# Khrylx/EgoPose

Measured on AMD Instinct MI355X. Metric: env-steps/sec (whole node) ego_mimic PPO, higher is better.
Workload: dtype f64 (rollout kernels K1-K6, physics state) + f32 (policy/value nets)

## Files before the change

egopose_amd/_lib.py:

```python
from __future__ import annotations

import ctypes as C
import os

HERE = os.path.dirname(os.path.abspath(__file__))
LIB_PATH = os.path.join(HERE, "libegopose_hip.so")

EGP_OK = 0
EGP_EXPERT_ROW = 168

c_int_p = C.POINTER(C.c_int32)
c_dbl_p = C.POINTER(C.c_double)
vp = C.c_void_p


class ModelDesc(C.Structure):
    _fields_ = [
        ("nq", C.c_int32), ("nv", C.c_int32), ("nu", C.c_int32), ("nbody", C.c_int32), ("nM", C.c_int32),
        ("body_qpos_start", c_int_p), ("body_ndof", c_int_p), ("dof_parentid", c_int_p), ("dof_Madr", c_int_p),
        ("ee_body", c_int_p),
        ("jkp", c_dbl_p), ("jkd", c_dbl_p), ("a_ref", c_dbl_p), ("a_scale", c_dbl_p), ("torque_lim", c_dbl_p),
        ("b_diffw", c_dbl_p),
        ("sub_dt", C.c_double), ("frame_skip", C.c_int32), ("episode_len", C.c_int32),
        ("w_p", C.c_double), ("w_v", C.c_double), ("w_e", C.c_double), ("w_rp", C.c_double), ("w_rv", C.c_double),
# ... 32 lines not shown
class MlpLayer(C.Structure):
    _fields_ = [("wt", vp), ("bias", vp), ("in_dim", C.c_int32), ("out_dim", C.c_int32)]


class GemmDesc(C.Structure):
    _fields_ = [("M", C.c_int32), ("N", C.c_int32), ("K", C.c_int32),
                ("A", vp), ("lda", C.c_int64), ("a_kcontig", C.c_int32),
                ("B", vp), ("ldb", C.c_int64), ("b_kcontig", C.c_int32),
                ("C", vp), ("ldc", C.c_int64),
                ("bias", vp), ("relu", C.c_int32),
                ("mask", vp), ("ldmask", C.c_int64),
                ("terms", C.c_int32), ("splits", C.c_int32), ("accumulate", C.c_int32),
                ("bias_grad", vp), ("workspace", vp),
                ("a_rows", vp), ("A2", vp), ("lda2", C.c_int64), ("a_split", C.c_int32), ("a_src_rows", C.c_int64),
                ("b_krows", vp), ("B2", vp), ("ldb2", C.c_int64), ("b_split", C.c_int32), ("b_src_rows", C.c_int64),
                ("c_rows", vp), ("a_krows", vp)]


class PpoLossDesc(C.Structure):
    _fields_ = [("n", C.c_int32), ("n_pol", C.c_int32), ("act_dim", C.c_int32),
                ("rows", vp), ("pred", vp), ("returns", vp),
                ("mean", vp), ("ld_mean", C.c_int64),
                ("actions", vp), ("ld_act", C.c_int64),
                ("log_std", vp), ("adv", vp),
                ("fixed_logp", vp), ("write_fixed", C.c_int32),
                ("clip_eps", C.c_double), ("inv_n_val", C.c_double), ("inv_n_exp", C.c_double),
                ("d_pred", vp), ("d_mean", vp), ("ld_dmean", C.c_int64), ("d_log_std", vp),
                ("losses", vp), ("workspace", vp)]


class MinibatchPlanDesc(C.Structure):
# ... 248 lines not shown
```

egopose_amd/csrc/egp_gemm.hip:

```cpp
#include "egp_internal.hpp"

#include <type_traits>

namespace {

typedef __bf16 bf16x8 __attribute__((ext_vector_type(8)));
typedef __bf16 bf16x4 __attribute__((ext_vector_type(4)));
typedef float f32x16 __attribute__((ext_vector_type(16)));
typedef float f32x4u __attribute__((ext_vector_type(4), aligned(4)));
typedef float f32x4 __attribute__((ext_vector_type(4)));
typedef float f32x2 __attribute__((ext_vector_type(2)));

inline int after_launch(const char *what) {
    hipError_t e = hipGetLastError();
    if (e != hipSuccess) {
        egp::set_error("launch of %s failed: %s", what, hipGetErrorString(e));
        return EGP_E_HIP;
    }
    return EGP_OK;
}

constexpr int BM = 128, BK = 32;

#ifdef EGP_GEMM_TRACE
// ... 20 lines not shown
#else
#define EGP_TR(tag) do { } while (0)
#define EGP_TRW_DECL do { } while (0)
#define EGP_TRW(who, tag) do { } while (0)
#endif
__host__ __device__ constexpr int panel_el(int R) { return R * 8 + 32; }
__host__ __device__ constexpr int tile_el(int R) { return 4 * panel_el(R); }

struct GemmArgs {
    int M, N, K;
    const float *A; long lda; int a_kc;
    const float *B; long ldb; int b_kc;
    float *C; long ldc;
    const float *bias; int relu;
    const float *mask; long ldmask;
    int ones_col;
    int k_per_split;
    float *ws; int ldws;
    int tiles_m, tiles_n, xcd_order;
    int split_xcd;
    const long long *a_rows; const float *A2; long lda2; int a_split;
    const long long *a_krows;
    const long long *b_krows; const float *B2; long ldb2; int b_split;
    const long long *c_rows;
    int partial;
    int grid_tiles, n_items, zs;
};

template <int R, bool ktail>
__device__ __forceinline__ void load_kc(const float *__restrict__ P, long ld, int rows, int r0, int k0, int kend, float (&v)[R / 8],
// ... 247 lines not shown
#pragma unroll
    for (int i = 0; i < MI; ++i)
#pragma unroll
        for (int j = 0; j < NJ; ++j) {
            const int col = n0 + wn * 64 + 32 * j + (lane & 31);
            const int rbase = m0 + wm * WROWS + 32 * i + 4 * (lane >> 5);
            const int colc = min(col, n_out - 1);
            const float bv = (!partial && g.bias) ? g.bias[min(colc, g.N - 1)] : 0.f;
            float keep[16];
            if (!partial && g.mask) {
#pragma unroll
                for (int r = 0; r < 16; ++r) {
                    const int row = min(rbase + (r & 3) + 8 * (r >> 2), g.M - 1);
                    keep[r] = g.mask[(long)row * g.ldmask + min(colc, g.N - 1)];
                }
            } else {
#pragma unroll
                for (int r = 0; r < 16; ++r) keep[r] = 1.f;
            }
            if (interior) {
#pragma unroll
                for (int r = 0; r < 16; ++r) {
                    const int row = rbase + (r & 3) + 8 * (r >> 2);
                    float x = partial ? acc[i][j][r] : fmaxf(acc[i][j][r] + bv, floor_v);
                    x = keep[r] > 0.f ? x : 0.f;
                    dst[(long)row * ldd + col] = x;
                }
            } else {
#pragma unroll
                for (int r = 0; r < 16; ++r) {
                    const int row = rbase + (r & 3) + 8 * (r >> 2);
                    float x = partial ? acc[i][j][r] : fmaxf(acc[i][j][r] + bv, floor_v);
                    x = keep[r] > 0.f ? x : 0.f;
                    if (row < g.M && col < n_out) dst[(long)row * ldd + col] = x;
                }
            }
        }
    EGP_TR(21);
}

struct WsCursor {
    int w, s, nst;
    int m0, n0, z, kbeg, kend;
};

template <int BN>
__device__ __forceinline__ bool ws_item(const GemmArgs &g, int w, WsCursor &c) {
    const int L = w % g.grid_tiles, z = w / g.grid_tiles;
    int tm, tn;
// ... 366 lines not shown
                    f32x16 a = acc[i][j];
                    a = __builtin_amdgcn_mfma_f32_32x32x16_bf16(fb[ks][0][j], fa[ks][2][i], a, 0, 0, 0);
                    a = __builtin_amdgcn_mfma_f32_32x32x16_bf16(fb[ks][2][j], fa[ks][0][i], a, 0, 0, 0);
                    a = __builtin_amdgcn_mfma_f32_32x32x16_bf16(fb[ks][1][j], fa[ks][1][i], a, 0, 0, 0);
                    a = __builtin_amdgcn_mfma_f32_32x32x16_bf16(fb[ks][0][j], fa[ks][1][i], a, 0, 0, 0);
                    a = __builtin_amdgcn_mfma_f32_32x32x16_bf16(fb[ks][1][j], fa[ks][0][i], a, 0, 0, 0);
                    acc[i][j] = __builtin_amdgcn_mfma_f32_32x32x16_bf16(fb[ks][0][j], fa[ks][0][i], a, 0, 0, 0);
                }
    };
    constexpr int EP_LD = 64 + 4;
    float *patch = (float *)(smem + (size_t)2 * BUF_EL * sizeof(__bf16)) + wave * 32 * EP_LD;
    const bool partial = g.partial != 0;
    const int ncols = partial ? g.ldws : g.N;
    const long ldd = partial ? g.ldws : g.ldc;
    const float floor_v = g.relu ? 0.f : -__builtin_inff();
    auto epilogue_body = [&](auto partial_c, auto mask_c) __attribute__((always_inline)) {
        constexpr bool PARTIAL = decltype(partial_c)::value, MASK = decltype(mask_c)::value;
        float *dst = PARTIAL ? g.ws + (long)cur.z * g.M * g.ldws : g.C;
        const int col = cur.n0 + wn * 64 + 4 * (lane & 15);
        const int colc = min(col, ncols - 4);
        const bool col_ok = col < ncols;
        const int row0 = cur.m0 + wm * WROWS + (lane >> 4);
        long drow[MI][8];
#pragma unroll
        for (int i = 0; i < MI; ++i)
#pragma unroll
            for (int it = 0; it < 8; ++it) {
                const int row = row0 + 32 * i + 4 * it;
                drow[i][it] = (FUSED && !PARTIAL && g.c_rows) ? (long)g.c_rows[min(row, g.M - 1)] : (long)row;
            }
        f32x4u bv = {0.f, 0.f, 0.f, 0.f};
        if constexpr (!PARTIAL) bv = *(const f32x4u *)((g.bias ? g.bias : g.C) + colc);
        if (PARTIAL || !g.bias) bv = f32x4u{0.f, 0.f, 0.f, 0.f};
        f32x4u keep[MI][8];
        if constexpr (MASK) {
#pragma unroll
            for (int i = 0; i < MI; ++i)
#pragma unroll
                for (int it = 0; it < 8; ++it)
                    keep[i][it] = *(const f32x4u *)(g.mask + (long)min(row0 + 32 * i + 4 * it, g.M - 1) * g.ldmask + colc);
        }
#pragma unroll
        for (int i = 0; i < MI; ++i) {
#pragma unroll
            for (int j = 0; j < NJ; ++j)
#pragma unroll
                for (int rq = 0; rq < 4; ++rq)
                    *(float4 *)(patch + (lane & 31) * EP_LD + 32 * j + 8 * rq + 4 * (lane >> 5)) =
                        make_float4(acc[i][j][4 * rq], acc[i][j][4 * rq + 1], acc[i][j][4 * rq + 2], acc[i][j][4 * rq + 3]);
            __builtin_amdgcn_wave_barrier();
#pragma unroll
            for (int it = 0; it < 8; ++it) {
                const int row = row0 + 32 * i + 4 * it;
                float4 x = *(const float4 *)(patch + ((lane >> 4) + 4 * it) * EP_LD + 4 * (lane & 15));
                if constexpr (!PARTIAL) {
                    x.x = fmaxf(x.x + bv[0], floor_v); x.y = fmaxf(x.y + bv[1], floor_v);
                    x.z = fmaxf(x.z + bv[2], floor_v); x.w = fmaxf(x.w + bv[3], floor_v);
                }
                if constexpr (MASK) {
                    x.x = keep[i][it][0] > 0.f ? x.x : 0.f; x.y = keep[i][it][1] > 0.f ? x.y : 0.f;
                    x.z = keep[i][it][2] > 0.f ? x.z : 0.f; x.w = keep[i][it][3] > 0.f ? x.w : 0.f;
                }
                if (row < g.M && col_ok) *(f32x4u *)(dst + drow[i][it] * ldd + col) = f32x4u{x.x, x.y, x.z, x.w};
            }
            __builtin_amdgcn_wave_barrier();
        }
    };
    auto epilogue = [&]() __attribute__((always_inline)) {
        if (partial) epilogue_body(std::true_type{}, std::false_type{});
        else if (g.mask) epilogue_body(std::false_type{}, std::true_type{});
        else epilogue_body(std::false_type{}, std::false_type{});
    };
    clear();
    __syncthreads();
    for (int p = 0; p < P; ++p) {
        EGP_TRW(0, 40);
#if !defined(EGP_WS_SKIP) || EGP_WS_SKIP != 1
        compute(p & 1);
#endif
        EGP_TRW(0, 41);
        if (cur.s == cur.nst - 1) {
            epilogue();
            EGP_TRW(0, 43);
            clear();
            EGP_TRW(0, 42);
        }
        ws_next<BN>(g, cur, w_scan);
        __syncthreads();
    }
}

__global__ __launch_bounds__(256) void k_gemv_rows(GemmArgs g) {
    const int lane = threadIdx.x & 63, wave = threadIdx.x >> 6;
    const long bs = g.b_kc ? 1 : g.ldb;
    const float floor_v = g.relu ? 0.f : -__builtin_inff();
    for (long m = (long)blockIdx.x * 4 + wave; m < g.M; m += (long)gridDim.x * 4) {
        const float *__restrict__ a = g.A + m * g.lda;
        float acc = 0.f;
        for (int k = lane; k < g.K; k += 64) acc = fmaf(a[k], g.B[k * bs], acc);
#pragma unroll
        for (int off = 32; off > 0; off >>= 1) acc += __shfl_down(acc, off, 64);
        if (lane == 0) {
            float x = fmaxf(acc + (g.bias ? g.bias[0] : 0.f), floor_v);
            if (g.mask && !(g.mask[m * g.ldmask] > 0.f)) x = 0.f;
            g.C[m * g.ldc] = x;
        }
    }
}

__global__ __launch_bounds__(256) void k_rank1(GemmArgs g) {
    const long as = g.a_kc ? g.lda : 1, bs = g.b_kc ? g.ldb : 1;
    const float floor_v = g.relu ? 0.f : -__builtin_inff();
    const long total = (long)g.M * g.N;
    for (long id = (long)blockIdx.x * 256 + threadIdx.x; id < total; id += (long)gridDim.x * 256) {
        const long m = id / g.N;
        const int n = (int)(id - m * g.N);
        float x = fmaxf(fmaf(g.A[m * as], g.B[n * bs], g.bias ? g.bias[n] : 0.f), floor_v);
        if (g.mask && !(g.mask[m * g.ldmask + n] > 0.f)) x = 0.f;
        g.C[m * g.ldc + n] = x;
    }
}

__global__ __launch_bounds__(256) void k_colsum(GemmArgs g) {
    __shared__ float s_part[4][256 + 4];
    const int lane = threadIdx.x & 63, wave = threadIdx.x >> 6, z = blockIdx.x;
    const long as = g.a_kc ? 1 : g.lda;
    const int kbeg = z * g.k_per_split, kend = min(g.K, kbeg + g.k_per_split);
    const int n_out = g.N + (g.ones_col ? 1 : 0);
    float *__restrict__ dst = g.ws + (long)z * g.ldws;
    for (int n0 = 0; n0 < g.N; n0 += 256) {
        float acc[4] = {0.f, 0.f, 0.f, 0.f};
        for (int k = kbeg + wave; k < kend; k += 32) {
            float a[8];
#pragma unroll
// ... 146 lines not shown
    if (splits <= 1 && !ones_col) return 0;
    return (int64_t)(splits < 1 ? 1 : splits) * M * ((N + (ones_col ? 1 : 0) + 3) & ~3);
}

int egp_gemm_f32(const egp_gemm_desc *d, void *stream) {
    EGP_REQUIRE(d, "descriptor is NULL");
    EGP_REQUIRE(d->M >= 0 && d->N >= 0 && d->K >= 0, "negative size");
    EGP_REQUIRE(d->terms == 1 || d->terms == 3 || d->terms == 6, "terms must be 1 (bf16), 3 (two-piece split) or 6 (three-piece split)");
    if (d->M == 0 || d->N + (d->bias_grad ? 1 : 0) == 0) return EGP_OK;
    EGP_REQUIRE(d->A && d->B && d->C, "NULL operand");
    const int ones = d->bias_grad ? 1 : 0;
    const int splits = d->splits < 1 ? 1 : d->splits;
    const bool partial = splits > 1 || ones;
    EGP_REQUIRE(!partial || d->workspace, "split-K / bias-gradient launches need a workspace (egp_gemm_workspace_floats)");
    EGP_REQUIRE(!partial || (!d->bias && !d->relu && !d->mask), "no epilogue on split-K launches");
    EGP_REQUIRE(!d->accumulate || partial, "accumulate goes with split-K / bias-gradient launches only (a plain product would overwrite C)");
    EGP_REQUIRE(!ones || !d->b_kcontig, "the ones column (bias gradient) goes with B given as [k][n]");
    hipStream_t s = (hipStream_t)stream;
    GemmArgs g;
    g.M = d->M; g.N = d->N; g.K = d->K;
    g.A = d->A; g.lda = d->lda; g.a_kc = d->a_kcontig;
    g.B = d->B; g.ldb = d->ldb; g.b_kc = d->b_kcontig;
    g.C = d->C; g.ldc = d->ldc;
    g.bias = d->bias; g.relu = d->relu; g.mask = d->mask; g.ldmask = d->ldmask;
    g.ones_col = ones; g.ws = d->workspace; g.ldws = (d->N + ones + 3) & ~3; g.partial = partial ? 1 : 0;
    g.a_rows = (const long long *)d->a_rows; g.A2 = d->A2; g.lda2 = d->lda2; g.a_split = d->a_split;
    g.b_krows = (const long long *)d->b_krows; g.B2 = d->B2; g.ldb2 = d->ldb2; g.b_split = d->b_split;
    g.c_rows = (const long long *)d->c_rows;
    g.a_krows = (const long long *)d->a_krows;
    const bool fused_io = d->a_rows || d->A2 || d->b_krows || d->B2 || d->c_rows || d->a_krows;
    if (fused_io) {
        EGP_REQUIRE(!(d->a_rows || d->A2) || d->a_kcontig, "a_rows / A2 go with a k-contiguous A");
        EGP_REQUIRE(!(d->b_krows || d->B2) || !d->b_kcontig, "b_krows / B2 go with B given as [k][n]");
        EGP_REQUIRE(!d->a_krows || !d->a_kcontig, "a_krows goes with A given as [k][m]");
        EGP_REQUIRE(!d->A2 || (d->a_split > 0 && d->a_split % BK == 0 && d->K - d->a_split >= BK),
                    "a_split must be a multiple of 32 and leave at least 32 columns to A2 (a k-tile reads one source)");
        EGP_REQUIRE(!d->A2 || splits == 1, "A2 does not go with split-K");
        EGP_REQUIRE(!d->B2 || (d->b_split > 0 && d->b_split % 128 == 0 && d->b_split < d->N + ones), "b_split must be a multiple of 128 inside (0, N)");
        EGP_REQUIRE(!d->B2 || d->N - d->b_split != 1 || d->K > BK, "a single-column B2 needs K > 32 (its first k-tile reads one element past each row)");
        EGP_REQUIRE(!d->c_rows || !partial, "c_rows (scatter) does not go with split-K / bias-gradient launches");
        EGP_REQUIRE(!d->a_rows || d->a_src_rows > 0, "a_rows needs a_src_rows (rows of the gathered source)");
        EGP_REQUIRE(!d->b_krows || d->b_src_rows > 0, "b_krows needs b_src_rows (rows of the gathered source)");
    }
    if (!fused_io) {
        if (d->N == 1 && !partial && d->a_kcontig && d->K >= 1) {
            const long blocks = std::min<long>(((long)d->M + 3) / 4, 256 * 16);
            k_gemv_rows<<<dim3((unsigned)blocks), dim3(256), 0, s>>>(g);
            return after_launch("k_gemv_rows");
        }
        if (d->K == 1 && !partial) {
            const long blocks = std::min<long>(((long)d->M * d->N + 255) / 256, 256 * 32);
            k_rank1<<<dim3((unsigned)blocks), dim3(256), 0, s>>>(g);
            return after_launch("k_rank1");
        }
        if (d->M == 1 && partial && !d->b_kcontig && d->K >= 1) {
            const int per_rows = (d->K + splits - 1) / splits;
            g.k_per_split = per_rows < 1 ? 1 : per_rows;
            const int zs1 = (d->K + g.k_per_split - 1) / g.k_per_split;
            k_colsum<<<dim3((unsigned)zs1), dim3(256), 0, s>>>(g);
            int rc1 = after_launch("k_colsum");
            if (rc1 != EGP_OK) return rc1;
            const int n_out1 = d->N + ones;
            k_gemm_reduce<<<dim3((unsigned)((n_out1 + 255) / 256)), dim3(256), 0, s>>>(d->workspace, g.ldws, zs1, 1, d->N, n_out1, d->C, d->ldc, d->bias_grad,
                                                                                    d->accumulate);
            return after_launch("k_gemm_reduce");
// ... 51 lines not shown
```

egopose_amd/gemm.py:

```python
from __future__ import annotations

import ctypes as C
import os

import torch

from . import _lib as L

_WS = {}


def enabled():
    return os.environ.get("EGP_GEMM", "hip") != "torch"


def default_terms():
    t = os.environ.get("EGP_GEMM_TERMS", "6")
    if t not in ("1", "3", "6"):
        raise ValueError("EGP_GEMM_TERMS must be 1, 3 or 6, got %r" % t)
    return int(t)


_WS_MAX = 8

# ... 30 lines not shown
    dev = torch.cuda.current_device() if device is None else int(device)
    if dev not in _CUS:
        n = int(L.load().egp_device_usable_cus(dev))
        _CUS[dev] = n if n > 0 else 256
    return _CUS[dev]


def pick_splits(M, n_out, K):
    cus = usable_cus()
    if M == 1:
        return max(1, min(cus, K // 128))
    tiles = ((M + 127) // 128) * ((n_out + 127) // 128)
    return max(1, min(cus // tiles, K // 256))


def _index(t, name):
    if not (t.is_cuda and t.dtype == torch.int64 and t.dim() == 1 and t.is_contiguous()):
        raise ValueError("%s must be a contiguous 1-D int64 HIP tensor" % name)
    return t


def gemm(A, B, a_kcontig=True, b_kcontig=True, bias=None, relu=False, mask=None, terms=None, splits=1, want_bias_grad=False,
         out=None, bias_grad_out=None, accumulate=False, a_rows=None, a2=None, b_krows=None, b2=None, c_rows=None, a_krows=None):
    A, B = _mat(A, "A"), _mat(B, "B")
    if accumulate and not (splits > 1 or want_bias_grad):
        raise ValueError("accumulate goes with splits > 1 or want_bias_grad (a plain product overwrites `out`)")
    M, K = (A.shape if a_kcontig else A.shape[::-1])
    N, Kb = (B.shape if b_kcontig else B.shape[::-1])
    a_split = b_split = 0
    if a_rows is not None or a2 is not None:
        if not a_kcontig:
            raise ValueError("a_rows / a2 go with a k-contiguous A")
        if a_rows is not None:
            M = _index(a_rows, "a_rows").shape[0]
        if a2 is not None:
            _mat(a2, "a2")
            if a2.shape[0] != M:
                raise ValueError("a2 has %d rows, the operand %d" % (a2.shape[0], M))
# ... 31 lines not shown
        d.b_krows, d.b_src_rows = b_krows.data_ptr(), B.shape[0]
    if b2 is not None:
        d.B2, d.ldb2, d.b_split = b2.data_ptr(), _ld(b2), b_split
    if c_rows is not None:
        d.c_rows = c_rows.data_ptr()
    if a_krows is not None:
        d.a_krows = a_krows.data_ptr()
    d.A, d.lda, d.a_kcontig = A.data_ptr(), _ld(A), 1 if a_kcontig else 0
    d.B, d.ldb, d.b_kcontig = B.data_ptr(), _ld(B), 1 if b_kcontig else 0
    d.C, d.ldc = out.data_ptr(), _ld(out)
    d.bias = bias.data_ptr() if bias is not None else None
    d.relu = 1 if relu else 0
    if mask is not None:
        _mat(mask, "mask")
        d.mask, d.ldmask = mask.data_ptr(), _ld(mask)
    d.terms = int(terms or default_terms())
    d.splits = int(splits)
    d.accumulate = 1 if accumulate else 0
    bg = None
    if want_bias_grad:
        bg = bias_grad_out if bias_grad_out is not None else torch.empty(M, dtype=torch.float32, device=dev)
        d.bias_grad = bg.data_ptr()
    if splits > 1 or want_bias_grad:
        ws = _workspace(L.load().egp_gemm_workspace_floats(M, N, 1 if want_bias_grad else 0, int(splits)), dev)
        d.workspace = ws.data_ptr()
    L.check(L.load().egp_gemm_f32(C.byref(d), L.current_stream()), "egp_gemm_f32")
    return (out, bg) if want_bias_grad else out


def linear_fwd(x, W, b=None, relu=False, terms=None):
    return gemm(x, W, True, True, bias=b, relu=relu, terms=terms)


def linear_dgrad(dy, W, mask=None, n_cols=None, terms=None):
    Wv = W if n_cols is None else W[:, :n_cols]
    return gemm(dy, Wv, True, False, mask=mask, terms=terms)


def linear_wgrad(dy, x, want_bias=True, terms=None):
    K, M = dy.shape
    n_out = x.shape[1] + (1 if want_bias else 0)
    return gemm(dy, x, False, False, terms=terms, splits=pick_splits(M, n_out, K), want_bias_grad=want_bias)


class MlpHead(torch.autograd.Function):

    @staticmethod
    def forward(ctx, x, n_grad_cols, *params):
        Ws, bs = params[0::2], params[1::2]
        hs = [x.contiguous()]
        for i, (W, b) in enumerate(zip(Ws, bs)):
            hs.append(linear_fwd(hs[-1], W.contiguous(), b, relu=i < len(Ws) - 1))
        ctx.save_for_backward(*hs[:-1], *Ws)
        ctx.n_layers, ctx.n_grad_cols = len(Ws), int(n_grad_cols)
        return hs[-1]

    @staticmethod
    def backward(ctx, dout):
        nl = ctx.n_layers
        hs, Ws = ctx.saved_tensors[:nl], ctx.saved_tensors[nl:]
        dz = dout.contiguous()
        grads = [None] * (2 * nl)
        dx = None
        for i in range(nl - 1, -1, -1):
            need_w, need_b = ctx.needs_input_grad[2 + 2 * i], ctx.needs_input_grad[3 + 2 * i]
            if need_w or need_b:
                dW, db = linear_wgrad(dz, hs[i], want_bias=True)
                grads[2 * i], grads[2 * i + 1] = (dW if need_w else None), (db if need_b else None)
            if i > 0:
                dz = linear_dgrad(dz, Ws[i].contiguous(), mask=hs[i])
            elif ctx.needs_input_grad[0]:
                nc = ctx.n_grad_cols
                W0 = Ws[0].contiguous()
                if nc >= W0.shape[1]:
                    dx = linear_dgrad(dz, W0)
                else:
                    dx = torch.zeros(dz.shape[0], W0.shape[1], dtype=dz.dtype, device=dz.device)
                    gemm(dz, W0[:, :nc], True, False, out=dx[:, :nc])
        return (dx, None, *grads)


def mlp_head_available(x, layers, head, activation):
    if isinstance(x, GatheredInput):
        x = x.x
    if not (enabled() and x.is_cuda and x.dtype == torch.float32 and x.dim() == 2 and activation is torch.relu):
        return False
    return all(l.weight.dtype == torch.float32 and l.bias is not None and l.weight.is_cuda for l in list(layers) + [head])


def mlp_head(x, layers, head, n_grad_cols=None):
    params = []
    for l in list(layers) + [head]:
        params += [l.weight, l.bias]
    nc = x.shape[1] if n_grad_cols is None else int(n_grad_cols)
    return MlpHead.apply(x, nc, *params)


class GatheredInput:

    def __init__(self, ctx2d, idx, x):
        self.ctx2d, self.idx, self.x = ctx2d, idx, x
        self.shape = (x.shape[0], ctx2d.shape[1] + x.shape[1])
        self.dtype, self.device, self.is_cuda = x.dtype, x.device, x.is_cuda

    def dim(self):
        return 2

    def size(self, k=None):
        return torch.Size(self.shape) if k is None else self.shape[k]

    def materialize(self):
        return GatherConcat.apply(self.ctx2d, self.idx, self.x)

    def __getitem__(self, ind):
        if torch.is_tensor(ind) and ind.dtype == torch.int64 and ind.dim() == 1:
            return GatheredInput(self.ctx2d, self.idx.index_select(0, ind), self.x.index_select(0, ind))
        return self.materialize()[ind]


def fused_gather_available(H, n_hidden, S):
    import os
    return enabled() and default_terms() == 6 and os.environ.get("EGP_GEMM_WS", "1") != "0" and H % 128 == 0 and n_hidden % 4 == 0 \
        and S >= 32


def fused_rows_available():
    import os
    return enabled() and default_terms() == 6 and os.environ.get("EGP_GEMM_WS", "1") != "0"


class GatherMlpHead(torch.autograd.Function):

    @staticmethod
    def forward(ctx, ctx2d, idx, x, *params):
        Ws, bs = params[0::2], params[1::2]
        ctx2d, x = ctx2d.contiguous(), (x if x.stride(1) == 1 else x.contiguous())
        h = gemm(ctx2d, Ws[0].contiguous(), True, True, bias=bs[0], relu=len(Ws) > 1, a_rows=idx, a2=x)
        hs = [h]
        for i in range(1, len(Ws)):
            hs.append(linear_fwd(hs[-1], Ws[i].contiguous(), bs[i], relu=i < len(Ws) - 1))
        ctx.save_for_backward(ctx2d, idx, x, *hs[:-1], *Ws)
        ctx.n_layers = len(Ws)
        return hs[-1]

    @staticmethod
    def backward(ctx, dout):
        nl = ctx.n_layers
        ctx2d, idx, x = ctx.saved_tensors[:3]
        hs, Ws = ctx.saved_tensors[3:3 + nl - 1], ctx.saved_tensors[3 + nl - 1:]
        dz = dout.contiguous()
        grads = [None] * (2 * nl)
        for i in range(nl - 1, 0, -1):
            need_w, need_b = ctx.needs_input_grad[3 + 2 * i], ctx.needs_input_grad[4 + 2 * i]
            if need_w or need_b:
                dW, db = linear_wgrad(dz, hs[i - 1], want_bias=True)
                grads[2 * i], grads[2 * i + 1] = (dW if need_w else None), (db if need_b else None)
            dz = linear_dgrad(dz, Ws[i].contiguous(), mask=hs[i - 1])
        H, S = ctx2d.shape[1], x.shape[1]
        if ctx.needs_input_grad[3] or ctx.needs_input_grad[4]:
            n = dz.shape[0]
            dW, db = gemm(dz, ctx2d, False, False, splits=pick_splits(dz.shape[1], H + S + 1, n), want_bias_grad=True, b_krows=idx, b2=x)
            grads[0], grads[1] = (dW if ctx.needs_input_grad[3] else None), (db if ctx.needs_input_grad[4] else None)
        dctx = None
        if ctx.needs_input_grad[0]:
            dctx = torch.zeros_like(ctx2d)
            gemm(dz, Ws[0][:, :H], True, False, out=dctx, c_rows=idx)
        return (dctx, None, None, *grads)


def gather_mlp_head(gi, layers, head):
    params = []
    for l in list(layers) + [head]:
        params += [l.weight, l.bias]
    return GatherMlpHead.apply(gi.ctx2d, gi.idx, gi.x, *params)


class GatherConcat(torch.autograd.Function):

    @staticmethod
    def forward(ctx, ctx2d, idx, x):
        n, H, S = idx.shape[0], ctx2d.shape[1], x.shape[1]
        out = torch.empty(n, H + S, dtype=torch.float32, device=x.device)
        L.check(L.load().egp_gather_concat_f32(ctx2d.data_ptr(), _ld(ctx2d), idx.data_ptr(), x.data_ptr(), _ld(x), n, H, S,
                                               out.data_ptr(), H + S, L.current_stream()), "egp_gather_concat_f32")
        ctx.save_for_backward(idx)
        ctx.shape = tuple(ctx2d.shape)
        return out

    @staticmethod
    def backward(ctx, dout):
        (idx,) = ctx.saved_tensors
        if not ctx.needs_input_grad[0]:
            return None, None, None
        R, H = ctx.shape
        dout = _mat(dout if dout.stride(1) == 1 else dout.contiguous(), "dout")
        dctx = torch.zeros(R, H, dtype=torch.float32, device=dout.device)
        L.check(L.load().egp_scatter_rows_f32(dout.data_ptr(), _ld(dout), idx.data_ptr(), idx.shape[0], H, dctx.data_ptr(), H,
                                              L.current_stream()), "egp_scatter_rows_f32")
        return dctx, None, None


def gather_concat_available(ctx2d, idx, x):
    return (enabled() and x.is_cuda and ctx2d.dtype == torch.float32 and x.dtype == torch.float32 and ctx2d.dim() == 2 and x.dim() == 2
            and ctx2d.is_contiguous() and x.stride(1) == 1 and idx.dtype == torch.int64 and idx.is_contiguous() and not x.requires_grad)
```

egopose_amd/nets.py:

```python
from __future__ import annotations

import math

import numpy as np
import torch
import torch.nn as nn

import os

from . import dist as _dist
from . import gemm as _gemm
from . import gemm_tuning as _tuning
from . import lstm as _hip_lstm
from . import tcn as _tcn
from .tcn import TemporalConvNet

_FWD_BUCKETS = 1
_LSTM_IMPL = os.environ.get("EGP_LSTM", "hip")

_ACT = {"tanh": torch.tanh, "relu": torch.relu, "sigmoid": torch.sigmoid}


def bucket_rows(x):
    if _tuning.enabled() and x.is_cuda and x.dim() == 2 and x.shape[0] >= 4 * _tuning.ROW_BUCKET:
# ... 249 lines not shown
        self.mode = "test"
        self.cnn_feat_dim, self.v_hdim, self.v_margin, self.v_net_type = cnn_feat_dim, v_hdim, v_margin, v_net_type
        self.v_net = _video_net(cnn_feat_dim, v_hdim, v_net_type, v_net_param, causal)
        self.v_out = None
        self.t = 0
        self.indices = None
        self.gather_indices = None
        self._gather_tm = None
        self._gather_unique = False
        self.cnn_feat_ctx = None
        self._buckets = None
        self._v_ctx = None
        self._ctx_key = None
        self._cnn_table = None
        self._ragged = None

    def set_mode(self, mode):
        self.mode = mode

    def forward_v_net(self, x):
        return _run_video_net(self.v_net, x)

    def attach_feature_table(self, table, take_offset):
        host = np.asarray(take_offset, dtype=np.int64)
        cur = getattr(self, "_cnn_table", None)
        if cur is not None and cur[0] is table and np.array_equal(getattr(self, "_take_offset_host", None), host):
            return
        self._cnn_table = (table, torch.as_tensor(host, dtype=torch.long, device=table.device))
        self._take_offset_host = host.copy()
        self._take_len = _take_lengths(take_offset, table.shape[0])
# ... 60 lines not shown
        lstm_ctx = self.cnn_feat_ctx.is_cuda and isinstance(self.v_net, RNN)
        self._ragged = _hip_lstm.ragged_order(steps, device, T=self.cnn_feat_ctx.shape[0]) if lstm_ctx else None
        self._buckets = None
        n_ep = len(ends)
        if _FWD_BUCKETS > 1 and n_ep >= 4 * _FWD_BUCKETS and self.v_net_type == "lstm":
            order = np.argsort(-lens, kind="stable")
            rank = np.empty(n_ep, np.int64)
            rank[order] = np.arange(n_ep)
            idx_s = np.arange(n)
            idx_s[:covered] = rank[ep_of] * max_len + (np.arange(covered) - np.repeat(starts, lens))
            self._gather_sorted = torch.as_tensor(idx_s, dtype=torch.long, device=device)
            self._ctx_sorted = self.cnn_feat_ctx.index_select(1, torch.as_tensor(order, device=device))
            cuts = [n_ep * k // _FWD_BUCKETS for k in range(_FWD_BUCKETS + 1)]
            lens_sorted = lens[order]
            self._buckets = [(cuts[k], cuts[k + 1], int(m + lens_sorted[cuts[k]])) for k in range(_FWD_BUCKETS)]

    _TRAIN_CONTEXT = ("indices", "cnn_feat_ctx", "gather_indices", "_gather_tm", "_gather_unique", "_ctx_key", "_ragged",
                      "_buckets", "_gather_sorted", "_ctx_sorted", "_frames")

    def adopt_train_context(self, other, x):
        alike = (isinstance(other, VideoStateNet) and self.mode == "train" and other.mode == "train" and other.cnn_feat_ctx is not None
                 and other._ctx_key is not None and self.v_margin == other.v_margin and self.cnn_feat_dim == other.cnn_feat_dim
                 and self.v_net_type == other.v_net_type and self._cnn_table is not None and other._cnn_table is not None
                 and self._cnn_table[0].data_ptr() == other._cnn_table[0].data_ptr()
                 and np.array_equal(self._take_offset_host, other._take_offset_host) and other.cnn_feat_ctx.dtype == x[0].dtype)
        if not alike:
            return self.initialize(x)
        for k in self._TRAIN_CONTEXT:
            if hasattr(other, k):
                setattr(self, k, getattr(other, k))

    def _bucketed_context(self):
        ctx, rnn = self._ctx_sorted, self.v_net
        T, B, _ = ctx.shape
        Hd = rnn.rnn_f.hidden_size
        out_f = ctx.new_zeros(T, B, Hd)
        for i0, i1, Tb in self._buckets:
            Tb = min(Tb, T)
            out_f[:Tb, i0:i1] = rnn._sweep(rnn.rnn_f, ctx[:Tb, i0:i1], False)
        if not rnn.bi_dir:
            return out_f
        return torch.cat((out_f, rnn._sweep(rnn.rnn_b, ctx, True)), 2)

    def forward(self, x, lazy_width=0):
        if self.mode == "test":
# ... 12 lines not shown
        if self._v_ctx is not None:
            (ctx, with_grad), self._v_ctx = self._v_ctx, None
            if with_grad != torch.is_grad_enabled():
                ctx = None
        if ctx is None and isinstance(self.v_net, RNN):
            self.v_net.ragged = self._ragged
            try:
                ctx = self.forward_v_net(self.cnn_feat_ctx)
            finally:
                self.v_net.ragged = None
        elif ctx is None:
            ctx = self.forward_v_net(self.cnn_feat_ctx)
        ctx2d = ctx.reshape(-1, self.v_hdim)
        if self._gather_unique and _gemm.gather_concat_available(ctx2d, self._gather_tm, x):
            if lazy_width and _gemm.fused_gather_available(self.v_hdim, lazy_width, x.shape[1]):
                return _gemm.GatheredInput(ctx2d, self._gather_tm, x)
            return tagged(_gemm.GatherConcat.apply(ctx2d, self._gather_tm, x))
        return tagged(torch.cat((ctx2d.index_select(0, self._gather_tm), x), dim=1))


class Bf16Shadow:

    def __init__(self, master):
        import copy
        self.master = master
        self.shadow = copy.deepcopy(master)
        for name, m in list(master.named_modules()):
            if isinstance(m, nn.modules.batchnorm._BatchNorm):
                parent = self.shadow
                *path, leaf = name.split(".")
                for part in path:
                    parent = getattr(parent, part)
# ... 316 lines not shown
```

include/egopose_hip.h:

```cpp
#ifndef EGOPOSE_HIP_H
#define EGOPOSE_HIP_H

#include <stdint.h>

#ifdef __cplusplus
extern "C" {
#endif

#define EGP_OK 0
#define EGP_E_INVALID (-1)
#define EGP_E_HIP (-2)
#define EGP_E_STATE (-3)
#define EGP_E_PHYSICS (-4)

#define EGP_MAX_NV 64
#define EGP_MAX_BODY 32
#define EGP_EXPERT_ROW 168

typedef struct egp_ctx egp_ctx;
typedef struct egp_physics egp_physics;
typedef struct egp_engine egp_engine;

typedef struct egp_model_desc {
    int32_t nq, nv, nu, nbody, nM;
// ... 120 lines not shown

typedef struct egp_gemm_desc {
    int32_t M, N, K;
    const float *A; int64_t lda; int32_t a_kcontig;
    const float *B; int64_t ldb; int32_t b_kcontig;
    float *C; int64_t ldc;
    const float *bias; int32_t relu;
    const float *mask; int64_t ldmask;
    int32_t terms, splits, accumulate;
    float *bias_grad;
    float *workspace;
    const int64_t *a_rows; const float *A2; int64_t lda2; int32_t a_split; int64_t a_src_rows;
    const int64_t *b_krows; const float *B2; int64_t ldb2; int32_t b_split; int64_t b_src_rows;
    const int64_t *c_rows;
    const int64_t *a_krows;
} egp_gemm_desc;
typedef struct egp_ppo_loss_desc {
    int32_t n, n_pol, act_dim;
    const int64_t *rows;
    const float *pred; const float *returns;
    const float *mean; int64_t ld_mean;
    const float *actions; int64_t ld_act;
    const float *log_std;
    const float *adv;
    float *fixed_logp; int32_t write_fixed;
    double clip_eps, inv_n_val, inv_n_exp;
    float *d_pred;
    float *d_mean; int64_t ld_dmean;
    float *d_log_std;
    double *losses;
// ... 263 lines not shown
```

Measured before the change: 1.008 million.

## Pack ReLU gates into bitmaps and reuse context-gradient buffers in MLP backward

The forward GEMM epilogue now emits a packed one-bit-per-element ReLU gate bitmap, and the backward data-gradient GEMM reads these bits instead of re-reading the full float hidden activation as a mask. This cuts mask read traffic in backward by a large factor. A row-vectorized rank-1 kernel is added for K==1 products. A pooled, lent buffer for the context gradient replaces per-call zero allocations. The cost is extra ballot and shuffle work plus bitmap stores in the forward epilogue, and extra bookkeeping for buffer lending.

```diff
diff --git a/egopose_amd/_lib.py b/egopose_amd/_lib.py
--- a/egopose_amd/_lib.py
+++ b/egopose_amd/_lib.py
@@ -70,7 +70,8 @@
                 ("bias_grad", vp), ("workspace", vp),
                 ("a_rows", vp), ("A2", vp), ("lda2", C.c_int64), ("a_split", C.c_int32), ("a_src_rows", C.c_int64),
                 ("b_krows", vp), ("B2", vp), ("ldb2", C.c_int64), ("b_split", C.c_int32), ("b_src_rows", C.c_int64),
-                ("c_rows", vp), ("a_krows", vp)]
+                ("c_rows", vp), ("a_krows", vp),
+                ("gate_out", vp), ("gate_bits", vp), ("ld_gate", C.c_int64)]
 
 
 class PpoLossDesc(C.Structure):
diff --git a/egopose_amd/csrc/egp_gemm.hip b/egopose_amd/csrc/egp_gemm.hip
--- a/egopose_amd/csrc/egp_gemm.hip
+++ b/egopose_amd/csrc/egp_gemm.hip
@@ -58,6 +58,7 @@
     float *C; long ldc;
     const float *bias; int relu;
     const float *mask; long ldmask;
+    unsigned *gate_out; const unsigned *gate_bits; long ld_gate;
     int ones_col;
     int k_per_split;
     float *ws; int ldws;
@@ -335,6 +336,13 @@
                     const int row = min(rbase + (r & 3) + 8 * (r >> 2), g.M - 1);
                     keep[r] = g.mask[(long)row * g.ldmask + min(colc, g.N - 1)];
                 }
+            } else if (!partial && g.gate_bits) {
+                const int cb = min(colc, g.N - 1);
+#pragma unroll
+                for (int r = 0; r < 16; ++r) {
+                    const int row = min(rbase + (r & 3) + 8 * (r >> 2), g.M - 1);
+                    keep[r] = (g.gate_bits[(long)row * g.ld_gate + (cb >> 5)] >> (cb & 31)) & 1u ? 1.f : 0.f;
+                }
             } else {
 #pragma unroll
                 for (int r = 0; r < 16; ++r) keep[r] = 1.f;
@@ -354,6 +362,18 @@
                     float x = partial ? acc[i][j][r] : fmaxf(acc[i][j][r] + bv, floor_v);
                     x = keep[r] > 0.f ? x : 0.f;
                     if (row < g.M && col < n_out) dst[(long)row * ldd + col] = x;
+                }
+            }
+            if (!partial && g.gate_out) {
+                const int wcol = n0 + wn * 64 + 32 * j;
+#pragma unroll
+                for (int r = 0; r < 16; ++r) {
+                    const int row = rbase + (r & 3) + 8 * (r >> 2);
+                    float x = fmaxf(acc[i][j][r] + bv, floor_v);
+                    x = keep[r] > 0.f ? x : 0.f;
+                    const unsigned long long b = __ballot(x > 0.f && col < g.N);
+                    const unsigned word = (lane >> 5) ? (unsigned)(b >> 32) : (unsigned)b;
+                    if ((lane & 31) == 0 && row < g.M && wcol < g.N) g.gate_out[(long)row * g.ld_gate + (wcol >> 5)] = word;
                 }
             }
         }
@@ -750,8 +770,23 @@
     const int ncols = partial ? g.ldws : g.N;
     const long ldd = partial ? g.ldws : g.ldc;
     const float floor_v = g.relu ? 0.f : -__builtin_inff();
-    auto epilogue_body = [&](auto partial_c, auto mask_c) __attribute__((always_inline)) {
-        constexpr bool PARTIAL = decltype(partial_c)::value, MASK = decltype(mask_c)::value;
+    constexpr int EPI_PLAIN = 0, EPI_MASK = 1, EPI_BITS = 2, EPI_GATE_OUT = 3;
+    unsigned gw[MI];
+#pragma unroll
+    for (int i = 0; i < MI; ++i) gw[i] = 0u;
+    auto gate_fetch = [&]() __attribute__((always_inline)) {
+        const int nwords = (g.N + 31) >> 5;
+        const int wi = min(((cur.n0 + wn * 64) >> 5) + (lane & 1), nwords - 1);
+#pragma unroll
+        for (int i = 0; i < MI; ++i) {
+            const int row = min(cur.m0 + wm * WROWS + 32 * i + (lane >> 1), g.M - 1);
+            gw[i] = g.gate_bits[(long)row * g.ld_gate + wi];
+        }
+    };
+    auto epilogue_body = [&](auto partial_c, auto epi_c) __attribute__((always_inline)) {
+        constexpr bool PARTIAL = decltype(partial_c)::value;
+        constexpr int EPI = decltype(epi_c)::value;
+        constexpr bool MASK = EPI == EPI_MASK;
         float *dst = PARTIAL ? g.ws + (long)cur.z * g.M * g.ldws : g.C;
         const int col = cur.n0 + wn * 64 + 4 * (lane & 15);
         const int colc = min(col, ncols - 4);
@@ -768,6 +803,32 @@
         f32x4u bv = {0.f, 0.f, 0.f, 0.f};
         if constexpr (!PARTIAL) bv = *(const f32x4u *)((g.bias ? g.bias : g.C) + colc);
         if (PARTIAL || !g.bias) bv = f32x4u{0.f, 0.f, 0.f, 0.f};
+        unsigned gword[NJ][MI];
+        if constexpr (EPI == EPI_GATE_OUT) {
+            f32x4u gb[NJ][4];
+#pragma unroll
+            for (int j = 0; j < NJ; ++j)
+#pragma unroll
+                for (int rq = 0; rq < 4; ++rq) {
+                    gb[j][rq] = *(const f32x4u *)((g.bias ? g.bias : g.C) + min(cur.n0 + wn * 64 + 32 * j + 8 * rq + 4 * (lane >> 5), ncols - 4));
+                    if (!g.bias) gb[j][rq] = f32x4u{0.f, 0.f, 0.f, 0.f};
+                }
+#pragma unroll
+            for (int j = 0; j < NJ; ++j)
+#pragma unroll
+                for (int i = 0; i < MI; ++i) {
+                    unsigned v = 0u;
+#pragma unroll
+                    for (int rq = 0; rq < 4; ++rq) {
+                        const bool qok = cur.n0 + wn * 64 + 32 * j + 8 * rq + 4 * (lane >> 5) < g.N;
+#pragma unroll
+                        for (int e = 0; e < 4; ++e)
+                            v |= (qok && acc[i][j][4 * rq + e] + gb[j][rq][e] > 0.f) ? 1u << (8 * rq + e) : 0u;
+                    }
+                    v <<= 4 * (lane >> 5);
+                    gword[j][i] = v | (unsigned)__shfl_xor((int)v, 32, 64);
+                }
+        }
         f32x4u keep[MI][8];
         if constexpr (MASK) {
 #pragma unroll
@@ -797,20 +858,39 @@
                     x.x = keep[i][it][0] > 0.f ? x.x : 0.f; x.y = keep[i][it][1] > 0.f ? x.y : 0.f;
                     x.z = keep[i][it][2] > 0.f ? x.z : 0.f; x.w = keep[i][it][3] > 0.f ? x.w : 0.f;
                 }
+                if constexpr (EPI == EPI_BITS) {
+                    const unsigned word = (unsigned)__shfl((int)gw[i], 2 * ((lane >> 4) + 4 * it) + ((lane >> 3) & 1), 64);
+                    const unsigned nib = word >> (4 * (lane & 7));
+                    x.x = (nib & 1u) ? x.x : 0.f; x.y = (nib & 2u) ? x.y : 0.f;
+                    x.z = (nib & 4u) ? x.z : 0.f; x.w = (nib & 8u) ? x.w : 0.f;
+                }
                 if (row < g.M && col_ok) *(f32x4u *)(dst + drow[i][it] * ldd + col) = f32x4u{x.x, x.y, x.z, x.w};
             }
             __builtin_amdgcn_wave_barrier();
+        }
+        if constexpr (EPI == EPI_GATE_OUT) {
+#pragma unroll
+            for (int j = 0; j < NJ; ++j)
+#pragma unroll
+                for (int i = 0; i < MI; ++i) {
+                    const int wcol = cur.n0 + wn * 64 + 32 * j;
+                    const int row = cur.m0 + wm * WROWS + 32 * i + (lane & 31);
+                    if (lane < 32 && row < g.M && wcol < g.N) g.gate_out[(long)row * g.ld_gate + (wcol >> 5)] = gword[j][i];
+                }
         }
     };
     auto epilogue = [&]() __attribute__((always_inline)) {
-        if (partial) epilogue_body(std::true_type{}, std::false_type{});
-        else if (g.mask) epilogue_body(std::false_type{}, std::true_type{});
-        else epilogue_body(std::false_type{}, std::false_type{});
+        if (partial) epilogue_body(std::true_type{}, std::integral_constant<int, EPI_PLAIN>{});
+        else if (g.mask) epilogue_body(std::false_type{}, std::integral_constant<int, EPI_MASK>{});
+        else if (g.gate_bits) epilogue_body(std::false_type{}, std::integral_constant<int, EPI_BITS>{});
+        else if (g.gate_out) epilogue_body(std::false_type{}, std::integral_constant<int, EPI_GATE_OUT>{});
+        else epilogue_body(std::false_type{}, std::integral_constant<int, EPI_PLAIN>{});
     };
     clear();
     __syncthreads();
     for (int p = 0; p < P; ++p) {
         EGP_TRW(0, 40);
+        if (g.gate_bits && cur.s == 0) gate_fetch();
 #if !defined(EGP_WS_SKIP) || EGP_WS_SKIP != 1
         compute(p & 1);
 #endif
@@ -839,6 +919,7 @@
         if (lane == 0) {
             float x = fmaxf(acc + (g.bias ? g.bias[0] : 0.f), floor_v);
             if (g.mask && !(g.mask[m * g.ldmask] > 0.f)) x = 0.f;
+            if (g.gate_bits && !(g.gate_bits[m * g.ld_gate] & 1u)) x = 0.f;
             g.C[m * g.ldc] = x;
         }
     }
@@ -853,7 +934,39 @@
         const int n = (int)(id - m * g.N);
         float x = fmaxf(fmaf(g.A[m * as], g.B[n * bs], g.bias ? g.bias[n] : 0.f), floor_v);
         if (g.mask && !(g.mask[m * g.ldmask + n] > 0.f)) x = 0.f;
+        if (g.gate_bits && !((g.gate_bits[m * g.ld_gate + (n >> 5)] >> (n & 31)) & 1u)) x = 0.f;
         g.C[m * g.ldc + n] = x;
+    }
+}
+
+__global__ __launch_bounds__(256) void k_rank1_rows(GemmArgs g) {
+    const int lane = threadIdx.x & 63, wave = threadIdx.x >> 6;
+    const long as = g.a_kc ? g.lda : 1;
+    const float floor_v = g.relu ? 0.f : -__builtin_inff();
+    const int nq = g.N >> 2;
+    for (int q0 = 0; q0 < nq; q0 += 64) {
+        const bool ok = q0 + lane < nq;
+        const int n = 4 * min(q0 + lane, nq - 1);
+        const f32x4u b = *(const f32x4u *)(g.B + n);
+        f32x4u bias = {0.f, 0.f, 0.f, 0.f};
+        if (g.bias) bias = *(const f32x4u *)(g.bias + n);
+        for (long m = (long)blockIdx.x * 4 + wave; m < g.M; m += (long)gridDim.x * 4) {
+            const float a = g.A[m * as];
+            f32x4u x;
+#pragma unroll
+            for (int e = 0; e < 4; ++e) x[e] = fmaxf(fmaf(a, b[e], bias[e]), floor_v);
+            if (g.mask) {
+                const f32x4u k = *(const f32x4u *)(g.mask + m * g.ldmask + n);
+#pragma unroll
+                for (int e = 0; e < 4; ++e) x[e] = k[e] > 0.f ? x[e] : 0.f;
+            }
+            if (g.gate_bits) {
+                const unsigned nib = g.gate_bits[m * g.ld_gate + (n >> 5)] >> (n & 31);
+#pragma unroll
+                for (int e = 0; e < 4; ++e) x[e] = (nib >> e) & 1u ? x[e] : 0.f;
+            }
+            if (ok) *(f32x4u *)(g.C + m * g.ldc + n) = x;
+        }
     }
 }
 
@@ -1030,6 +1143,12 @@
     const bool partial = splits > 1 || ones;
     EGP_REQUIRE(!partial || d->workspace, "split-K / bias-gradient launches need a workspace (egp_gemm_workspace_floats)");
     EGP_REQUIRE(!partial || (!d->bias && !d->relu && !d->mask), "no epilogue on split-K launches");
+    EGP_REQUIRE(!partial || (!d->gate_out && !d->gate_bits), "gate_out / gate_bits do not go with split-K / bias-gradient launches");
+    EGP_REQUIRE(!d->c_rows || (!d->gate_out && !d->gate_bits), "gate_out / gate_bits do not go with c_rows (the bitmap follows the product's rows)");
+    EGP_REQUIRE(!d->gate_bits || !d->mask, "gate_bits and mask are the same gate twice: give one");
+    EGP_REQUIRE(!d->gate_bits || !d->gate_out, "gate_out goes with a forward product, gate_bits with a data gradient");
+    EGP_REQUIRE(!(d->gate_out || d->gate_bits) || d->ld_gate >= ((int64_t)d->N + 31) / 32, "ld_gate < ceil(N / 32) words");
+    EGP_REQUIRE(!d->gate_out || (d->N != 1 && d->K != 1), "gate_out is not written by the thin products (N == 1 or K == 1)");
     EGP_REQUIRE(!d->accumulate || partial, "accumulate goes with split-K / bias-gradient launches only (a plain product would overwrite C)");
     EGP_REQUIRE(!ones || !d->b_kcontig, "the ones column (bias gradient) goes with B given as [k][n]");
     hipStream_t s = (hipStream_t)stream;
@@ -1039,6 +1158,7 @@
     g.B = d->B; g.ldb = d->ldb; g.b_kc = d->b_kcontig;
     g.C = d->C; g.ldc = d->ldc;
     g.bias = d->bias; g.relu = d->relu; g.mask = d->mask; g.ldmask = d->ldmask;
+    g.gate_out = d->gate_out; g.gate_bits = d->gate_bits; g.ld_gate = d->ld_gate;
     g.ones_col = ones; g.ws = d->workspace; g.ldws = (d->N + ones + 3) & ~3; g.partial = partial ? 1 : 0;
     g.a_rows = (const long long *)d->a_rows; g.A2 = d->A2; g.lda2 = d->lda2; g.a_split = d->a_split;
     g.b_krows = (const long long *)d->b_krows; g.B2 = d->B2; g.ldb2 = d->ldb2; g.b_split = d->b_split;
@@ -1065,6 +1185,11 @@
             return after_launch("k_gemv_rows");
         }
         if (d->K == 1 && !partial) {
+            if (d->N % 4 == 0 && (d->b_kcontig ? d->ldb == 1 : true)) {
+                const long row_blocks = std::min<long>(((long)d->M + 3) / 4, 256 * 16);
+                k_rank1_rows<<<dim3((unsigned)row_blocks), dim3(256), 0, s>>>(g);
+                return after_launch("k_rank1_rows");
+            }
             const long blocks = std::min<long>(((long)d->M * d->N + 255) / 256, 256 * 32);
             k_rank1<<<dim3((unsigned)blocks), dim3(256), 0, s>>>(g);
             return after_launch("k_rank1");
diff --git a/egopose_amd/gemm.py b/egopose_amd/gemm.py
--- a/egopose_amd/gemm.py
+++ b/egopose_amd/gemm.py
@@ -2,6 +2,7 @@
 
 import ctypes as C
 import os
+import weakref
 
 import torch
 
@@ -68,6 +69,16 @@
     return max(1, min(cus // tiles, K // 256))
 
 
+def gate_bitmap(M, N, device, ld_gate=None):
+    return torch.empty(M, (N + 31) // 32 if ld_gate is None else int(ld_gate), dtype=torch.int32, device=device)
+
+
+def _gate(t, M, N, name):
+    if not (t.is_cuda and t.dtype == torch.int32 and t.dim() == 2 and t.shape[0] >= M and t.shape[1] * 32 >= N and (t.shape[1] == 1 or t.stride(1) == 1)):
+        raise ValueError("%s must be a 2-D int32 HIP tensor of at least (%d, %d) words, got %s %s" % (name, M, (N + 31) // 32, tuple(t.shape), t.dtype))
+    return t.data_ptr(), _ld(t)
+
+
 def _index(t, name):
     if not (t.is_cuda and t.dtype == torch.int64 and t.dim() == 1 and t.is_contiguous()):
         raise ValueError("%s must be a contiguous 1-D int64 HIP tensor" % name)
@@ -75,7 +86,8 @@
 
 
 def gemm(A, B, a_kcontig=True, b_kcontig=True, bias=None, relu=False, mask=None, terms=None, splits=1, want_bias_grad=False,
-         out=None, bias_grad_out=None, accumulate=False, a_rows=None, a2=None, b_krows=None, b2=None, c_rows=None, a_krows=None):
+         out=None, bias_grad_out=None, accumulate=False, a_rows=None, a2=None, b_krows=None, b2=None, c_rows=None, a_krows=None,
+         gate_out=None, gate_bits=None):
     A, B = _mat(A, "A"), _mat(B, "B")
     if accumulate and not (splits > 1 or want_bias_grad):
         raise ValueError("accumulate goes with splits > 1 or want_bias_grad (a plain product overwrites `out`)")
@@ -137,6 +149,10 @@
     if mask is not None:
         _mat(mask, "mask")
         d.mask, d.ldmask = mask.data_ptr(), _ld(mask)
+    if gate_out is not None:
+        d.gate_out, d.ld_gate = _gate(gate_out, M, N, "gate_out")
+    if gate_bits is not None:
+        d.gate_bits, d.ld_gate = _gate(gate_bits, M, N, "gate_bits")
     d.terms = int(terms or default_terms())
     d.splits = int(splits)
     d.accumulate = 1 if accumulate else 0
@@ -151,13 +167,13 @@
     return (out, bg) if want_bias_grad else out
 
 
-def linear_fwd(x, W, b=None, relu=False, terms=None):
-    return gemm(x, W, True, True, bias=b, relu=relu, terms=terms)
-
-
-def linear_dgrad(dy, W, mask=None, n_cols=None, terms=None):
+def linear_fwd(x, W, b=None, relu=False, terms=None, gate_out=None):
+    return gemm(x, W, True, True, bias=b, relu=relu, terms=terms, gate_out=gate_out)
+
+
+def linear_dgrad(dy, W, mask=None, n_cols=None, terms=None, gate_bits=None):
     Wv = W if n_cols is None else W[:, :n_cols]
-    return gemm(dy, Wv, True, False, mask=mask, terms=terms)
+    return gemm(dy, Wv, True, False, mask=mask, terms=terms, gate_bits=gate_bits)
 
 
 def linear_wgrad(dy, x, want_bias=True, terms=None):
@@ -172,16 +188,20 @@
     def forward(ctx, x, n_grad_cols, *params):
         Ws, bs = params[0::2], params[1::2]
         hs = [x.contiguous()]
+        gates = []
         for i, (W, b) in enumerate(zip(Ws, bs)):
-            hs.append(linear_fwd(hs[-1], W.contiguous(), b, relu=i < len(Ws) - 1))
-        ctx.save_for_backward(*hs[:-1], *Ws)
+            hidden = i < len(Ws) - 1
+            if hidden:
+                gates.append(gate_bitmap(x.shape[0], W.shape[0], x.device))
+            hs.append(linear_fwd(hs[-1], W.contiguous(), b, relu=hidden, gate_out=gates[-1] if hidden else None))
+        ctx.save_for_backward(*hs[:-1], *Ws, *gates)
         ctx.n_layers, ctx.n_grad_cols = len(Ws), int(n_grad_cols)
         return hs[-1]
 
     @staticmethod
     def backward(ctx, dout):
         nl = ctx.n_layers
-        hs, Ws = ctx.saved_tensors[:nl], ctx.saved_tensors[nl:]
+        hs, Ws, gates = ctx.saved_tensors[:nl], ctx.saved_tensors[nl:2 * nl], ctx.saved_tensors[2 * nl:]
         dz = dout.contiguous()
         grads = [None] * (2 * nl)
         dx = None
@@ -191,7 +211,7 @@
                 dW, db = linear_wgrad(dz, hs[i], want_bias=True)
                 grads[2 * i], grads[2 * i + 1] = (dW if need_w else None), (db if need_b else None)
             if i > 0:
-                dz = linear_dgrad(dz, Ws[i].contiguous(), mask=hs[i])
+                dz = linear_dgrad(dz, Ws[i].contiguous(), gate_bits=gates[i - 1])
             elif ctx.needs_input_grad[0]:
                 nc = ctx.n_grad_cols
                 W0 = Ws[0].contiguous()
@@ -219,10 +239,36 @@
     return MlpHead.apply(x, nc, *params)
 
 
+class _DctxLoan:
+    __slots__ = ("buf", "done", "__weakref__")
+
+    def __init__(self, buf):
+        self.buf, self.done = buf, False
+
+
+class ContextGradBuffer:
+
+    def __init__(self, rows, width, device, dtype=torch.float32):
+        self.buf = torch.zeros(rows, width, dtype=dtype, device=device)
+        self._loan = None
+
+    def lend(self, ctx2d):
+        if not (torch.is_grad_enabled() and ctx2d.requires_grad and ctx2d.shape == self.buf.shape and ctx2d.dtype == self.buf.dtype
+                and ctx2d.device == self.buf.device):
+            return None
+        prev = self._loan() if self._loan is not None else None
+        if prev is not None and not prev.done:
+            return None
+        loan = _DctxLoan(self.buf)
+        self._loan = weakref.ref(loan)
+        return loan
+
+
 class GatheredInput:
 
-    def __init__(self, ctx2d, idx, x):
+    def __init__(self, ctx2d, idx, x, dctx=None):
         self.ctx2d, self.idx, self.x = ctx2d, idx, x
+        self.dctx = dctx
         self.shape = (x.shape[0], ctx2d.shape[1] + x.shape[1])
         self.dtype, self.device, self.is_cuda = x.dtype, x.device, x.is_cuda
 
@@ -232,8 +278,12 @@
     def size(self, k=None):
         return torch.Size(self.shape) if k is None else self.shape[k]
 
+    def take_dctx(self):
+        loan, self.dctx = self.dctx, None
+        return loan
+
     def materialize(self):
-        return GatherConcat.apply(self.ctx2d, self.idx, self.x)
+        return GatherConcat.apply(self.ctx2d, self.idx, self.x, self.take_dctx())
 
     def __getitem__(self, ind):
         if torch.is_tensor(ind) and ind.dtype == torch.int64 and ind.dim() == 1:
@@ -255,72 +305,83 @@
 class GatherMlpHead(torch.autograd.Function):
 
     @staticmethod
-    def forward(ctx, ctx2d, idx, x, *params):
+    def forward(ctx, ctx2d, idx, x, dctx, *params):
         Ws, bs = params[0::2], params[1::2]
         ctx2d, x = ctx2d.contiguous(), (x if x.stride(1) == 1 else x.contiguous())
-        h = gemm(ctx2d, Ws[0].contiguous(), True, True, bias=bs[0], relu=len(Ws) > 1, a_rows=idx, a2=x)
+        n = idx.shape[0]
+        gates = [gate_bitmap(n, W.shape[0], x.device) for W in Ws[:-1]]
+        h = gemm(ctx2d, Ws[0].contiguous(), True, True, bias=bs[0], relu=len(Ws) > 1, a_rows=idx, a2=x, gate_out=gates[0] if gates else None)
         hs = [h]
         for i in range(1, len(Ws)):
-            hs.append(linear_fwd(hs[-1], Ws[i].contiguous(), bs[i], relu=i < len(Ws) - 1))
-        ctx.save_for_backward(ctx2d, idx, x, *hs[:-1], *Ws)
+            hidden = i < len(Ws) - 1
+            hs.append(linear_fwd(hs[-1], Ws[i].contiguous(), bs[i], relu=hidden, gate_out=gates[i] if hidden else None))
+        ctx.save_for_backward(ctx2d, idx, x, *hs[:-1], *Ws, *gates)
         ctx.n_layers = len(Ws)
+        ctx.dctx = dctx
         return hs[-1]
 
     @staticmethod
     def backward(ctx, dout):
         nl = ctx.n_layers
         ctx2d, idx, x = ctx.saved_tensors[:3]
-        hs, Ws = ctx.saved_tensors[3:3 + nl - 1], ctx.saved_tensors[3 + nl - 1:]
+        hs, Ws = ctx.saved_tensors[3:3 + nl - 1], ctx.saved_tensors[3 + nl - 1:3 + 2 * nl - 1]
+        gates = ctx.saved_tensors[3 + 2 * nl - 1:]
         dz = dout.contiguous()
         grads = [None] * (2 * nl)
         for i in range(nl - 1, 0, -1):
-            need_w, need_b = ctx.needs_input_grad[3 + 2 * i], ctx.needs_input_grad[4 + 2 * i]
+            need_w, need_b = ctx.needs_input_grad[4 + 2 * i], ctx.needs_input_grad[5 + 2 * i]
             if need_w or need_b:
                 dW, db = linear_wgrad(dz, hs[i - 1], want_bias=True)
                 grads[2 * i], grads[2 * i + 1] = (dW if need_w else None), (db if need_b else None)
-            dz = linear_dgrad(dz, Ws[i].contiguous(), mask=hs[i - 1])
+            dz = linear_dgrad(dz, Ws[i].contiguous(), gate_bits=gates[i - 1])
         H, S = ctx2d.shape[1], x.shape[1]
-        if ctx.needs_input_grad[3] or ctx.needs_input_grad[4]:
+        if ctx.needs_input_grad[4] or ctx.needs_input_grad[5]:
             n = dz.shape[0]
             dW, db = gemm(dz, ctx2d, False, False, splits=pick_splits(dz.shape[1], H + S + 1, n), want_bias_grad=True, b_krows=idx, b2=x)
-            grads[0], grads[1] = (dW if ctx.needs_input_grad[3] else None), (db if ctx.needs_input_grad[4] else None)
+            grads[0], grads[1] = (dW if ctx.needs_input_grad[4] else None), (db if ctx.needs_input_grad[5] else None)
         dctx = None
         if ctx.needs_input_grad[0]:
-            dctx = torch.zeros_like(ctx2d)
+            dctx = ctx.dctx.buf if ctx.dctx is not None else torch.zeros_like(ctx2d)
             gemm(dz, Ws[0][:, :H], True, False, out=dctx, c_rows=idx)
-        return (dctx, None, None, *grads)
+        if ctx.dctx is not None:
+            ctx.dctx.done = True
+        return (dctx, None, None, None, *grads)
 
 
 def gather_mlp_head(gi, layers, head):
     params = []
     for l in list(layers) + [head]:
         params += [l.weight, l.bias]
-    return GatherMlpHead.apply(gi.ctx2d, gi.idx, gi.x, *params)
+    return GatherMlpHead.apply(gi.ctx2d, gi.idx, gi.x, gi.take_dctx(), *params)
 
 
 class GatherConcat(torch.autograd.Function):
 
     @staticmethod
-    def forward(ctx, ctx2d, idx, x):
+    def forward(ctx, ctx2d, idx, x, dctx=None):
         n, H, S = idx.shape[0], ctx2d.shape[1], x.shape[1]
         out = torch.empty(n, H + S, dtype=torch.float32, device=x.device)
         L.check(L.load().egp_gather_concat_f32(ctx2d.data_ptr(), _ld(ctx2d), idx.data_ptr(), x.data_ptr(), _ld(x), n, H, S,
                                                out.data_ptr(), H + S, L.current_stream()), "egp_gather_concat_f32")
         ctx.save_for_backward(idx)
         ctx.shape = tuple(ctx2d.shape)
+        ctx.dctx = dctx
+        ctx.n_inputs = len(ctx.needs_input_grad)
         return out
 
     @staticmethod
     def backward(ctx, dout):
         (idx,) = ctx.saved_tensors
+        if ctx.dctx is not None:
+            ctx.dctx.done = True
         if not ctx.needs_input_grad[0]:
-            return None, None, None
+            return (None,) * ctx.n_inputs
         R, H = ctx.shape
         dout = _mat(dout if dout.stride(1) == 1 else dout.contiguous(), "dout")
-        dctx = torch.zeros(R, H, dtype=torch.float32, device=dout.device)
+        dctx = ctx.dctx.buf if ctx.dctx is not None else torch.zeros(R, H, dtype=torch.float32, device=dout.device)
         L.check(L.load().egp_scatter_rows_f32(dout.data_ptr(), _ld(dout), idx.data_ptr(), idx.shape[0], H, dctx.data_ptr(), H,
                                               L.current_stream()), "egp_scatter_rows_f32")
-        return dctx, None, None
+        return (dctx,) + (None,) * (ctx.n_inputs - 1)
 
 
 def gather_concat_available(ctx2d, idx, x):
diff --git a/egopose_amd/nets.py b/egopose_amd/nets.py
--- a/egopose_amd/nets.py
+++ b/egopose_amd/nets.py
@@ -287,6 +287,7 @@
         self._ctx_key = None
         self._cnn_table = None
         self._ragged = None
+        self._dctx_buf = None
 
     def set_mode(self, mode):
         self.mode = mode
@@ -377,9 +378,19 @@
             cuts = [n_ep * k // _FWD_BUCKETS for k in range(_FWD_BUCKETS + 1)]
             lens_sorted = lens[order]
             self._buckets = [(cuts[k], cuts[k + 1], int(m + lens_sorted[cuts[k]])) for k in range(_FWD_BUCKETS)]
+        self._new_dctx_buf()
 
     _TRAIN_CONTEXT = ("indices", "cnn_feat_ctx", "gather_indices", "_gather_tm", "_gather_unique", "_ctx_key", "_ragged",
                       "_buckets", "_gather_sorted", "_ctx_sorted", "_frames")
+
+    def _new_dctx_buf(self):
+        self._dctx_buf = None
+        c = self.cnn_feat_ctx
+        if c is not None and c.is_cuda and c.dtype == torch.float32 and self._gather_unique and self._buckets is None and _gemm.enabled():
+            self._dctx_buf = _gemm.ContextGradBuffer(c.shape[0] * c.shape[1], self.v_hdim, c.device)
+
+    def _lend_dctx_buf(self, ctx2d):
+        return self._dctx_buf.lend(ctx2d) if self._dctx_buf is not None else None
 
     def adopt_train_context(self, other, x):
         alike = (isinstance(other, VideoStateNet) and self.mode == "train" and other.mode == "train" and other.cnn_feat_ctx is not None
@@ -392,6 +403,7 @@
         for k in self._TRAIN_CONTEXT:
             if hasattr(other, k):
                 setattr(self, k, getattr(other, k))
+        self._new_dctx_buf()
 
     def _bucketed_context(self):
         ctx, rnn = self._ctx_sorted, self.v_net
@@ -434,8 +446,8 @@
         ctx2d = ctx.reshape(-1, self.v_hdim)
         if self._gather_unique and _gemm.gather_concat_available(ctx2d, self._gather_tm, x):
             if lazy_width and _gemm.fused_gather_available(self.v_hdim, lazy_width, x.shape[1]):
-                return _gemm.GatheredInput(ctx2d, self._gather_tm, x)
-            return tagged(_gemm.GatherConcat.apply(ctx2d, self._gather_tm, x))
+                return _gemm.GatheredInput(ctx2d, self._gather_tm, x, self._lend_dctx_buf(ctx2d))
+            return tagged(_gemm.GatherConcat.apply(ctx2d, self._gather_tm, x, self._lend_dctx_buf(ctx2d)))
         return tagged(torch.cat((ctx2d.index_select(0, self._gather_tm), x), dim=1))
 
 
diff --git a/include/egopose_hip.h b/include/egopose_hip.h
--- a/include/egopose_hip.h
+++ b/include/egopose_hip.h
@@ -158,6 +158,7 @@
     const int64_t *b_krows; const float *B2; int64_t ldb2; int32_t b_split; int64_t b_src_rows;
     const int64_t *c_rows;
     const int64_t *a_krows;
+    uint32_t *gate_out; const uint32_t *gate_bits; int64_t ld_gate;
 } egp_gemm_desc;
 typedef struct egp_ppo_loss_desc {
     int32_t n, n_pol, act_dim;
```

New measurement: 997,600. -1.0%, worse.
